# PaddlePaddle/PaddleNLP

Measured on AMD Instinct MI355X. Metric: tokens_per_sec_whole_node_llama3_8b_pretrain, higher is better.
Workload: dtype bf16; 1 GPU; model=llama3-8b, global_batch=8, seq_len=4096, parallelism=single, recompute=False

## Files before the change

### paddlenlp_amd/ops/csrc/flash_attn_bwd_v2.hip

```cpp
#include "launchers.h"
#include "mfma.h"

#define FB2_WAVES 8
#define FB2_BLOCK (FB2_WAVES * 64)

template <int D, bool MASKED = false>
__global__ __launch_bounds__(FB2_BLOCK) void flash_bwd2_dq_kernel(
    const ushort_t* __restrict__ q, const ushort_t* __restrict__ k,
    const ushort_t* __restrict__ v, const ushort_t* __restrict__ dout,
    const float* __restrict__ lse, const float* __restrict__ delta,
    ushort_t* __restrict__ dq, const int* __restrict__ startend,
    FlashStrides rs,
    int B, int Sq, int Skv, int Hq, int Hk, float scale, int causal) {
    constexpr int BLKN = 64;
    constexpr int DSTEPS = D / 16;
    constexpr int NDT = D / 32;
    constexpr int BLKM = FB2_WAVES * 32;

    __shared__ ushort_t k_lds[2][BLKN * D];
    __shared__ ushort_t v_lds[2][BLKN * D];
    __shared__ ushort_t kt_lds[2][D * BLKN];
    __shared__ int se_lds[2][MASKED ? BLKN : 1];

    const int tid = threadIdx.x;
    const int wave = tid >> 6;
    const int lane = tid & 63;
    const int l32 = lane & 31;
    const int hi = lane >> 5;

    int qt, bh;
    xcd_grouped_tile<FA_ORDER_W, false>(qt, bh);
    const int b = bh / Hq, hq = bh % Hq;
    const int hk = hq / (Hq / Hk);
    const int q_base = qt * BLKM;
    const int qw = q_base + wave * 32;
    const int qg = qw + l32;
    const int causal_off = Skv - Sq;

    const long long q_row_stride = rs.q;
    const long long kv_row_stride = rs.kv;
    const long long do_row_stride = (long long)Hq * D;
    const ushort_t* q_ptr = q + (long long)b * Sq * q_row_stride + (long long)hq * D;
    const ushort_t* do_ptr = dout + ((long long)b * Sq * Hq + hq) * D;
    const ushort_t* k_ptr = k + (long long)b * Skv * kv_row_stride + (long long)hk * D;
    const ushort_t* v_ptr = v + (long long)b * Skv * kv_row_stride + (long long)hk * D;

    frag8 aq[DSTEPS], ado[DSTEPS];
    float lse_q = INFINITY, dl_q = 0.f;
    if (qg < Sq) {
#pragma unroll
        for (int kk = 0; kk < DSTEPS; kk++) {
            aq[kk] = *reinterpret_cast<const frag8*>(
                q_ptr + (long long)qg * q_row_stride + kk * 16 + hi * 8);
            ado[kk] = *reinterpret_cast<const frag8*>(
                do_ptr + (long long)qg * do_row_stride + kk * 16 + hi * 8);
        }
        lse_q = lse[((long long)b * Hq + hq) * Sq + qg];
        dl_q = delta[((long long)b * Hq + hq) * Sq + qg];
    } else {
#pragma unroll
        for (int kk = 0; kk < DSTEPS; kk++) { aq[kk] = frag8{0}; ado[kk] = frag8{0}; }
    }

    f32x16 acc_dq[NDT];
#pragma unroll
    for (int n = 0; n < NDT; n++)
#pragma unroll
        for (int r = 0; r < 16; r++) acc_dq[n][r] = 0.f;

    int n_kv_tiles = (Skv + BLKN - 1) / BLKN;
    if (causal) {
        int max_kv = q_base + BLKM - 1 + causal_off;
        int lim = (max_kv + BLKN) / BLKN;
        n_kv_tiles = min(n_kv_tiles, max(lim, 0));
    }

    const int s_rowp = tid >> 4;
    const int s_col = (tid & 15) * 8;
    const int s_row0 = s_rowp * 2;
    short8v sk0, sk1, sv0, sv1;

    auto load_tile = [&](int kv_base) {
        int g0 = kv_base + s_row0;
        sk0 = short8v{0,0,0,0,0,0,0,0}; sk1 = sk0; sv0 = sk0; sv1 = sk0;
        if (g0 < Skv) {
            sk0 = *reinterpret_cast<const short8v*>(k_ptr + (long long)g0 * kv_row_stride + s_col);
            sv0 = *reinterpret_cast<const short8v*>(v_ptr + (long long)g0 * kv_row_stride + s_col);
        }
        if (g0 + 1 < Skv) {
            sk1 = *reinterpret_cast<const short8v*>(k_ptr + (long long)(g0 + 1) * kv_row_stride + s_col);
            sv1 = *reinterpret_cast<const short8v*>(v_ptr + (long long)(g0 + 1) * kv_row_stride + s_col);
        }
    };
    auto write_tile = [&](int buf, int kv_base) {
        if (MASKED && tid < BLKN) {
            int g = kv_base + tid;
            se_lds[buf][tid] =
                (g < Skv) ? startend[(long long)b * Skv + g] : 0;
        }
        *reinterpret_cast<short8v*>(swz<D>(k_lds[buf], s_row0, s_col)) = sk0;
        *reinterpret_cast<short8v*>(swz<D>(k_lds[buf], s_row0 + 1, s_col)) = sk1;
        *reinterpret_cast<short8v*>(swz<D>(v_lds[buf], s_row0, s_col)) = sv0;
        *reinterpret_cast<short8v*>(swz<D>(v_lds[buf], s_row0 + 1, s_col)) = sv1;
#pragma unroll
        for (int j = 0; j < 8; j++) {
            unsigned p32 = ((unsigned)(unsigned short)sk0[j]) |
                           (((unsigned)(unsigned short)sk1[j]) << 16);
            *reinterpret_cast<unsigned*>(swz<BLKN>(kt_lds[buf], s_col + j, s_row0)) = p32;
        }
    };

    auto tile_se_max = [&](int kv_base) -> int {
        int g = kv_base + lane;
        int v = (g < Skv) ? startend[(long long)b * Skv + g] : 0;
#pragma unroll
        for (int off = 32; off; off >>= 1)
            v = max(v, __shfl_xor(v, off, 64));
        return v;
    };

    load_tile(0);
    write_tile(0, 0);
    int se_max_cur = MASKED ? tile_se_max(0) : 0x7fffffff;
    __syncthreads();

    for (int kvt = 0; kvt < n_kv_tiles; kvt++) {
        const int kv_base = kvt * BLKN;
        const int cur = kvt & 1;
        bool wave_skip =
            causal && (kv_base > qw + 31 + causal_off);
        if (MASKED && qw >= se_max_cur) wave_skip = true;

        auto process_sub = [&](int sub) {
            f32x16 st, dp;
#pragma unroll
            for (int r = 0; r < 16; r++) { st[r] = 0.f; dp[r] = 0.f; }
            __builtin_amdgcn_s_setprio(1);
#pragma unroll
            for (int kk = 0; kk < DSTEPS; kk++) {
                frag8 ak = *reinterpret_cast<const frag8*>(
                    swz<D>(k_lds[cur], sub * 32 + l32, kk * 16 + hi * 8));
                frag8 av = *reinterpret_cast<const frag8*>(
                    swz<D>(v_lds[cur], sub * 32 + l32, kk * 16 + hi * 8));
                st = mfma32(ak, aq[kk], st);
                dp = mfma32(av, ado[kk], dp);
            }
            __builtin_amdgcn_s_setprio(0);

#pragma unroll
            for (int r = 0; r < 16; r++) {
                int row = sub * 32 + crow32(r, hi);
                int kvg = kv_base + row;
                bool vis = (kvg < Skv) && (qg < Sq) &&
                           (!causal || kvg <= qg + causal_off);
                if (MASKED) vis = vis && (qg < se_lds[cur][row]);
                float p = vis ? __expf(st[r] * scale - lse_q) : 0.f;
                st[r] = p * (dp[r] - dl_q) * scale;
            }

            __builtin_amdgcn_s_setprio(1);
#pragma unroll
            for (int ksl = 0; ksl < 2; ksl++) {
                const int ks = sub * 2 + ksl;
                frag8 ads = t12_convert(st, ksl * 8);
#pragma unroll
                for (int n = 0; n < NDT; n++) {
                    frag8 bkf = *reinterpret_cast<const frag8*>(
                        swz<BLKN>(kt_lds[cur], n * 32 + l32, ks * 16 + hi * 8));
                    acc_dq[n] = mfma32(ads, bkf, acc_dq[n]);
                }
            }
            __builtin_amdgcn_s_setprio(0);
        };

        if (!wave_skip) process_sub(0);
        int se_max_next = 0x7fffffff;
        bool stage_skip = false;
        if (kvt + 1 < n_kv_tiles) {
            if (MASKED) {
                se_max_next = tile_se_max(kv_base + BLKN);
                stage_skip = (q_base >= se_max_next);
            }
            if (!stage_skip) load_tile(kv_base + BLKN);
        }
        if (!wave_skip) process_sub(1);

        if (kvt + 1 < n_kv_tiles && !stage_skip)
            write_tile(cur ^ 1, kv_base + BLKN);
        if (MASKED) se_max_cur = se_max_next;
        __syncthreads();
    }

#pragma unroll
    for (int r = 0; r < 16; r++) {
        int qrow = qw + crow32(r, hi);
        if (qrow >= Sq) continue;
        ushort_t* dqr = dq + ((long long)b * Sq + qrow) * rs.dq + (long long)hq * D;
#pragma unroll
        for (int n = 0; n < NDT; n++)
            dqr[n * 32 + l32] = f32_to_bf16(acc_dq[n][r]);
    }
}

template <int D, bool MASKED = false>
__global__ __launch_bounds__(FB2_BLOCK, 1) void flash_bwd2_dkv_kernel(
    const ushort_t* __restrict__ q, const ushort_t* __restrict__ k,
    const ushort_t* __restrict__ v, const ushort_t* __restrict__ dout,
    const float* __restrict__ lse, const float* __restrict__ delta,
    ushort_t* __restrict__ dk, ushort_t* __restrict__ dv,
    const int* __restrict__ startend,
    FlashStrides rs,
    int B, int Sq, int Skv, int Hq, int Hk, float scale, int causal) {
    static_assert(D == 128, "the dual-use image is laid out for 128-column tiles");
    constexpr int BLKQ = 64;
    constexpr int DSTEPS = D / 16;
    constexpr int NDT = D / 32;
    constexpr int BLKKV = FB2_WAVES * 32;

    __shared__ __attribute__((aligned(16))) ushort_t qd_lds[2][2][BLKQ * D];
    __shared__ float ld_lds[2][2][BLKQ];

    const int tid = threadIdx.x;
    const int wave = __builtin_amdgcn_readfirstlane(tid >> 6);
    const int lane = tid & 63;
    const int l32 = lane & 31;
    const int hi = lane >> 5;

    int kvt, bh;
    xcd_grouped_tile<FA_ORDER_W, true>(kvt, bh);
    const int b = bh / Hk, hk = bh % Hk;
    const int G = Hq / Hk;
    const int kv_base = kvt * BLKKV;
    const int kvw = kv_base + wave * 32;
    const int kvg_lane = kvw + l32;
    const int causal_off = Skv - Sq;
    __shared__ int blk_max_lds[MASKED ? FB2_WAVES : 1];
    int kv_end_lane = 0x7fffffff;
    int wave_max_end = 0x7fffffff;
    if (MASKED) {
        kv_end_lane = (kvg_lane < Skv)
            ? startend[(long long)b * Skv + kvg_lane] : 0;
        wave_max_end = kv_end_lane;
#pragma unroll
        for (int off = 32; off; off >>= 1)
            wave_max_end = max(wave_max_end,
                               __shfl_xor(wave_max_end, off, 64));
        wave_max_end = __builtin_amdgcn_readfirstlane(wave_max_end);
        if (lane == 0) blk_max_lds[wave] = wave_max_end;
    }

    const long long do_row_stride = (long long)Hq * D;
    const ushort_t* k_ptr = k + (long long)b * Skv * rs.kv + (long long)hk * D;
    const ushort_t* v_ptr = v + (long long)b * Skv * rs.kv + (long long)hk * D;

    frag8 bk[DSTEPS], bv[DSTEPS];
    if (kvg_lane < Skv) {
#pragma unroll
        for (int kk = 0; kk < DSTEPS; kk++) {
            bk[kk] = *reinterpret_cast<const frag8*>(
                k_ptr + (long long)kvg_lane * rs.kv + kk * 16 + hi * 8);
            bv[kk] = *reinterpret_cast<const frag8*>(
                v_ptr + (long long)kvg_lane * rs.kv + kk * 16 + hi * 8);
        }
    } else {
#pragma unroll
        for (int kk = 0; kk < DSTEPS; kk++) { bk[kk] = frag8{0}; bv[kk] = frag8{0}; }
    }

    f32x16 acc_dk[NDT], acc_dv[NDT];
#pragma unroll
    for (int n = 0; n < NDT; n++)
#pragma unroll
        for (int r = 0; r < 16; r++) { acc_dk[n][r] = 0.f; acc_dv[n][r] = 0.f; }

    int qt0 = 0;
    if (causal) qt0 = max(0, (kv_base - causal_off) / BLKQ);
    int qt_end = (Sq + BLKQ - 1) / BLKQ;
    if (MASKED) {
        __syncthreads();
        int block_max_end = blk_max_lds[0];
#pragma unroll
        for (int w = 1; w < FB2_WAVES; w++)
            block_max_end = max(block_max_end, blk_max_lds[w]);
        block_max_end = __builtin_amdgcn_readfirstlane(block_max_end);
        if (block_max_end < Sq)
            qt_end = (max(block_max_end, 0) + BLKQ - 1) / BLKQ;
    }
    const int n_tiles = G * max(qt_end - qt0, 0);

    auto issue_tile = [&](int g, int qt, int buf) {
        const int hq = hk * G + g;
        const long long do_off = ((long long)b * Sq * Hq + hq) * D;
        const long long q_off = (long long)b * Sq * rs.q + (long long)hq * D;
        const int q_tb = qt * BLKQ;
        const int ln = fresh_lane_id();
#pragma unroll
        for (int i = 0; i < 2; i++) {
            const int piece = wave * 2 + i;
            const int src_row = min(q_tb + img_fill_row(piece, ln), Sq - 1);
            const int chunk = img_fill_chunk(piece, ln) * 8;
            lds_dma16(q + (q_off + (long long)src_row * rs.q + chunk),
                      &qd_lds[buf][0][piece * 512]);
            lds_dma16(dout + (do_off + (long long)src_row * do_row_stride + chunk),
                      &qd_lds[buf][1][piece * 512]);
        }
        if (wave < 2) {
            const float* row = (wave == 0 ? lse : delta) +
                               ((long long)b * Hq + hq) * Sq;
            lds_dma4(row + min(q_tb + ln, Sq - 1), &ld_lds[buf][wave][0]);
        }
    };

    int g_next = 0, qt_next = qt0;
    auto advance_next = [&]() {
        if (++qt_next == qt_end) { qt_next = qt0; g_next++; }
    };
#pragma unroll
    for (int kk = 0; kk < DSTEPS; kk++)
        asm volatile("" :: "v"(bk[kk]), "v"(bv[kk]));
    if (n_tiles > 0) { issue_tile(g_next, qt_next, 0); advance_next(); }

    int qt = qt0;
    for (int t = 0; t < n_tiles; t++) {
        const int cur = t & 1;
        lds_dma_wait_all();
        __syncthreads();
        if (t + 1 < n_tiles) { issue_tile(g_next, qt_next, cur ^ 1); advance_next(); }

        const int q_tb = qt * BLKQ;
        const ushort_t* q_img = qd_lds[cur][0];
        const ushort_t* do_img = qd_lds[cur][1];
        const int lane_t = fresh_lane_id();
        bool wave_skip =
            causal && (q_tb + BLKQ - 1 + causal_off < kvw);
        if (MASKED && q_tb >= wave_max_end) wave_skip = true;

        if (!wave_skip) {
#pragma unroll 1
            for (int sub = 0; sub < 2; sub++) {
                f32x16 st, dp;
#pragma unroll
                for (int r = 0; r < 16; r++) { st[r] = 0.f; dp[r] = 0.f; }
                __builtin_amdgcn_s_setprio(1);
#pragma unroll
                for (int kk = 0; kk < DSTEPS; kk++) {
                    frag8 aqf = img_row_frag(q_img, sub * 32 + l32, kk, hi);
                    frag8 adf = img_row_frag(do_img, sub * 32 + l32, kk, hi);
                    st = mfma32(aqf, bk[kk], st);
                    dp = mfma32(adf, bv[kk], dp);
                }
                __builtin_amdgcn_s_setprio(0);

#pragma unroll
                for (int r = 0; r < 16; r++) {
                    int qrow = sub * 32 + crow32(r, hi);
                    int qgl = q_tb + qrow;
                    float ls = ld_lds[cur][0][qrow];
                    float dl = ld_lds[cur][1][qrow];
                    bool vis = (qgl < Sq) && (kvg_lane < Skv) &&
                               (!causal || kvg_lane <= qgl + causal_off);
                    if (MASKED) vis = vis && (qgl < kv_end_lane);
                    float p = (vis && ls != INFINITY)
                                  ? __expf(st[r] * scale - ls) : 0.f;
                    st[r] = p;
                    dp[r] = p * (dp[r] - dl) * scale;
                }

                __builtin_amdgcn_s_setprio(1);
#pragma unroll
                for (int ksl = 0; ksl < 2; ksl++) {
                    const int ks = sub * 2 + ksl;
                    frag8 apt = t12_convert(st, ksl * 8);
                    frag8 ads = t12_convert(dp, ksl * 8);
#pragma unroll
                    for (int n = 0; n < NDT; n++) {
                        frag8 bdo = img_tr_frag(do_img, ks, n, lane_t);
                        frag8 bq = img_tr_frag(q_img, ks, n, lane_t);
                        acc_dv[n] = mfma32(apt, bdo, acc_dv[n]);
                        acc_dk[n] = mfma32(ads, bq, acc_dk[n]);
                    }
                }
                __builtin_amdgcn_s_setprio(0);
            }
        }
        if (++qt == qt_end) qt = qt0;
    }

#pragma unroll
    for (int r = 0; r < 16; r++) {
        int kvr = kvw + crow32(r, hi);
        if (kvr >= Skv) continue;
        long long base = ((long long)b * Skv + kvr) * rs.dkv + (long long)hk * D;
#pragma unroll
        for (int n = 0; n < NDT; n++) {
            dk[base + n * 32 + l32] = f32_to_bf16(acc_dk[n][r]);
            dv[base + n * 32 + l32] = f32_to_bf16(acc_dv[n][r]);
        }
    }
}

__global__ __launch_bounds__(64) void lds_image_probe(
    const ushort_t* __restrict__ X, ushort_t* __restrict__ out_row,
    ushort_t* __restrict__ out_tr) {
    __shared__ __attribute__((aligned(16))) ushort_t img[64 * 128];
    const int lane = threadIdx.x;
    const int l32 = lane & 31, hi = lane >> 5;
#pragma unroll 1
    for (int piece = 0; piece < 16; piece++)
        lds_dma16(X + img_fill_row(piece, lane) * 128 + img_fill_chunk(piece, lane) * 8,
                  &img[piece * 512]);
    lds_dma_wait_all();
    __syncthreads();
    for (int sub = 0; sub < 2; sub++)
        for (int kk = 0; kk < 8; kk++) {
            frag8 f = img_row_frag(img, sub * 32 + l32, kk, hi);
            *reinterpret_cast<frag8*>(
                out_row + (sub * 32 + l32) * 128 + kk * 16 + hi * 8) = f;
        }
    for (int ks = 0; ks < 4; ks++)
        for (int n = 0; n < 4; n++) {
            frag8 f = img_tr_frag(img, ks, n, lane);
#pragma unroll
            for (int j = 0; j < 8; j++)
                out_tr[(ks * 16 + hi * 8 + j) * 128 + n * 32 + l32] = (ushort_t)f[j];
        }
}

void launch_lds_image_probe(const void* X, void* out_row, void* out_tr,
                            hipStream_t stream) {
    hipLaunchKernelGGL(lds_image_probe, dim3(1), dim3(64), 0, stream,
                       (const ushort_t*)X, (ushort_t*)out_row, (ushort_t*)out_tr);
}

bool launch_flash_bwd2(const void* dout, const void* q, const void* k, const void* v,
                       const void* o, const float* lse, float* delta,
                       void* dq, void* dk, void* dv,
                       int B, int Sq, int Skv, int Hq, int Hk, int D,
                       float scale, bool causal, hipStream_t stream, int parts,
                       const FlashStrides* strides) {
    if (D != 128 || (Hq % Hk) != 0) return false;
    const FlashStrides rs = strides ? *strides : flash_contiguous_strides(Hq, Hk, D);
    if (parts & FLASH_BWD_DELTA)
        launch_flash_bwd_delta(dout, o, delta, B, Sq, Hq, D, stream);
    if (parts & FLASH_BWD_DQ) {
        dim3 gq((Sq + 255) / 256, B * Hq);
        hipLaunchKernelGGL((flash_bwd2_dq_kernel<128, false>), gq, dim3(FB2_BLOCK), 0, stream,
                           (const ushort_t*)q, (const ushort_t*)k, (const ushort_t*)v,
                           (const ushort_t*)dout, lse, delta, (ushort_t*)dq,
                           (const int*)nullptr, rs,
                           B, Sq, Skv, Hq, Hk, scale, causal ? 1 : 0);
    }
    if (parts & FLASH_BWD_DKV) {
        dim3 gkv((Skv + 255) / 256, B * Hk);
        hipLaunchKernelGGL((flash_bwd2_dkv_kernel<128, false>), gkv, dim3(FB2_BLOCK), 0, stream,
                           (const ushort_t*)q, (const ushort_t*)k, (const ushort_t*)v,
                           (const ushort_t*)dout, lse, delta, (ushort_t*)dk, (ushort_t*)dv,
                           (const int*)nullptr, rs,
                           B, Sq, Skv, Hq, Hk, scale, causal ? 1 : 0);
    }
    return true;
}

bool launch_flash_bwd2_mask(const void* dout, const void* q, const void* k,
                            const void* v, const void* o, const float* lse,
                            float* delta, void* dq, void* dk, void* dv,
                            const int* startend,
                            int B, int Sq, int Skv, int Hq, int Hk, int D,
                            float scale, hipStream_t stream,
                            const FlashStrides* strides) {
    if (D != 128 || (Hq % Hk) != 0) return false;
    const FlashStrides rs = strides ? *strides : flash_contiguous_strides(Hq, Hk, D);
    launch_flash_bwd_delta(dout, o, delta, B, Sq, Hq, D, stream);
    dim3 gq((Sq + 255) / 256, B * Hq);
    hipLaunchKernelGGL((flash_bwd2_dq_kernel<128, true>), gq, dim3(FB2_BLOCK), 0, stream,
                       (const ushort_t*)q, (const ushort_t*)k, (const ushort_t*)v,
                       (const ushort_t*)dout, lse, delta, (ushort_t*)dq, startend, rs,
                       B, Sq, Skv, Hq, Hk, scale, 1);
    dim3 gkv((Skv + 255) / 256, B * Hk);
    hipLaunchKernelGGL((flash_bwd2_dkv_kernel<128, true>), gkv, dim3(FB2_BLOCK), 0, stream,
                       (const ushort_t*)q, (const ushort_t*)k, (const ushort_t*)v,
                       (const ushort_t*)dout, lse, delta, (ushort_t*)dk, (ushort_t*)dv,
                       startend, rs, B, Sq, Skv, Hq, Hk, scale, 1);
    return true;
}
```

### paddlenlp_amd/ops/csrc/flash_attn_v2.hip

```cpp
#include "launchers.h"
#include "mfma.h"

#define FA2_WAVES 8
#define FA2_BLOCK (FA2_WAVES * 64)
#define FA2_BLKN 64
#define FA2_QW 32
#define FA2_BLKM (FA2_WAVES * FA2_QW)
#define DEFER_THR 8.0f

__global__ void mfma32_layout_probe(const ushort_t* A, const ushort_t* B, float* C) {
    int l = threadIdx.x;
    int l32 = l & 31, hi = l >> 5;
    frag8 a, b;
#pragma unroll
    for (int j = 0; j < 8; j++) {
        a[j] = (short)A[l32 * 16 + hi * 8 + j];
        b[j] = (short)B[(hi * 8 + j) * 32 + l32];
    }
    f32x16 c;
#pragma unroll
    for (int r = 0; r < 16; r++) c[r] = 0.f;
    c = mfma32(a, b, c);
#pragma unroll
    for (int r = 0; r < 16; r++) C[crow32(r, hi) * 32 + l32] = c[r];
}

__global__ void permlane_probe(int* out0, int* out1) {
    int l = threadIdx.x;
    auto r = __builtin_amdgcn_permlane32_swap((unsigned)l, (unsigned)(1000 + l),
                                              false, false);
    out0[l] = (int)r[0];
    out1[l] = (int)r[1];
}

template <int D, bool MASKED = false>
__global__ __launch_bounds__(FA2_BLOCK) void flash_fwd2_kernel(
    const ushort_t* __restrict__ q,
    const ushort_t* __restrict__ k,
    const ushort_t* __restrict__ v,
    ushort_t* __restrict__ o,
    float* __restrict__ lse,
    const int* __restrict__ startend,
    FlashStrides rs,
    int B, int Sq, int Skv, int Hq, int Hk, float scale, int causal) {
    constexpr int DSTEPS = D / 16;
    constexpr int NDT = D / 32;
    constexpr int KVT = FA2_BLKN / 32;

    __shared__ ushort_t k_lds[2][FA2_BLKN * D];
    __shared__ ushort_t vt_lds[2][D * FA2_BLKN];
    __shared__ int se_lds[2][MASKED ? FA2_BLKN : 1];

    const int tid = threadIdx.x;
    const int wave = tid >> 6;
    const int lane = tid & 63;
    const int l32 = lane & 31;
    const int hi = lane >> 5;

    int qt, bh;
    xcd_grouped_tile<FA_ORDER_W, false>(qt, bh);
    const int b = bh / Hq, hq = bh % Hq;
    const int hk = hq / (Hq / Hk);
    const int q_base = qt * FA2_BLKM;
    const int qw = q_base + wave * FA2_QW;
    const int qg = qw + l32;
    const int causal_off = Skv - Sq;

    const long long q_row_stride = rs.q;
    const long long kv_row_stride = rs.kv;
    const long long o_row_stride = (long long)Hq * D;
    const ushort_t* q_ptr = q + (long long)b * Sq * q_row_stride + (long long)hq * D;
    const ushort_t* k_ptr = k + (long long)b * Skv * kv_row_stride + (long long)hk * D;
    const ushort_t* v_ptr = v + (long long)b * Skv * kv_row_stride + (long long)hk * D;

    frag8 aq[DSTEPS];
    if (qg < Sq) {
#pragma unroll
        for (int kk = 0; kk < DSTEPS; kk++)
            aq[kk] = *reinterpret_cast<const frag8*>(
                q_ptr + (long long)qg * q_row_stride + kk * 16 + hi * 8);
    } else {
#pragma unroll
        for (int kk = 0; kk < DSTEPS; kk++) aq[kk] = frag8{0};
    }

    float m_run = -INFINITY, l_run = 0.f;
    f32x16 acc_o[NDT];
#pragma unroll
    for (int n = 0; n < NDT; n++)
#pragma unroll
        for (int r = 0; r < 16; r++) acc_o[n][r] = 0.f;

    int n_kv_tiles = (Skv + FA2_BLKN - 1) / FA2_BLKN;
    if (causal) {
        int max_kv = q_base + FA2_BLKM - 1 + causal_off;
        int lim = (max_kv + FA2_BLKN) / FA2_BLKN;
        n_kv_tiles = min(n_kv_tiles, max(lim, 0));
    }

    const int s_rowp = tid >> 4;
    const int s_col = (tid & 15) * 8;
    const int s_row0 = s_rowp * 2;
    short8v sk0, sk1, sv0, sv1;

    auto load_tile = [&](int kv_base) {
        int g0 = kv_base + s_row0;
        sk0 = short8v{0,0,0,0,0,0,0,0}; sk1 = sk0; sv0 = sk0; sv1 = sk0;
        if (g0 < Skv) {
            sk0 = *reinterpret_cast<const short8v*>(k_ptr + (long long)g0 * kv_row_stride + s_col);
            sv0 = *reinterpret_cast<const short8v*>(v_ptr + (long long)g0 * kv_row_stride + s_col);
        }
        if (g0 + 1 < Skv) {
            sk1 = *reinterpret_cast<const short8v*>(k_ptr + (long long)(g0 + 1) * kv_row_stride + s_col);
            sv1 = *reinterpret_cast<const short8v*>(v_ptr + (long long)(g0 + 1) * kv_row_stride + s_col);
        }
    };
    auto write_tile = [&](int buf, int kv_base) {
        if (MASKED && tid < FA2_BLKN) {
            int g = kv_base + tid;
            se_lds[buf][tid] =
                (g < Skv) ? startend[(long long)b * Skv + g] : 0;
        }
        *reinterpret_cast<short8v*>(swz<D>(k_lds[buf], s_row0, s_col)) = sk0;
        *reinterpret_cast<short8v*>(swz<D>(k_lds[buf], s_row0 + 1, s_col)) = sk1;
#pragma unroll
        for (int j = 0; j < 8; j++) {
            unsigned p32 = ((unsigned)(unsigned short)sv0[j]) |
                           (((unsigned)(unsigned short)sv1[j]) << 16);
            *reinterpret_cast<unsigned*>(swz<FA2_BLKN>(vt_lds[buf], s_col + j, s_row0)) = p32;
        }
    };

    auto tile_bounds = [&](int kv_base, int& mn_out) -> int {
        int g = kv_base + lane;
        int v = (g < Skv) ? startend[(long long)b * Skv + g] : 0;
        int mx = v, mn = (g < Skv) ? v : 0x7fffffff;
#pragma unroll
        for (int off = 32; off; off >>= 1) {
            mx = max(mx, __shfl_xor(mx, off, 64));
            mn = min(mn, __shfl_xor(mn, off, 64));
        }
        mn_out = mn;
        return mx;
    };

    load_tile(0);
    write_tile(0, 0);
    int se_min_cur = 0, se_max_cur = 0x7fffffff;
    if (MASKED) se_max_cur = tile_bounds(0, se_min_cur);
    __syncthreads();

    for (int kvt = 0; kvt < n_kv_tiles; kvt++) {
        const int kv_base = kvt * FA2_BLKN;
        const int cur = kvt & 1;
        bool wave_skip =
            causal && (kv_base > qw + FA2_QW - 1 + causal_off);
        if (MASKED && qw >= se_max_cur) wave_skip = true;

        f32x16 st[KVT];
        if (!wave_skip) {
#pragma unroll
            for (int nt = 0; nt < KVT; nt++)
#pragma unroll
                for (int r = 0; r < 16; r++) st[nt][r] = 0.f;
            __builtin_amdgcn_s_setprio(1);
#pragma unroll
            for (int kk = 0; kk < DSTEPS; kk++) {
#pragma unroll
                for (int nt = 0; nt < KVT; nt++) {
                    frag8 ak = *reinterpret_cast<const frag8*>(
                        swz<D>(k_lds[cur], nt * 32 + l32, kk * 16 + hi * 8));
                    st[nt] = mfma32(ak, aq[kk], st[nt]);
                }
            }
            __builtin_amdgcn_s_setprio(0);
        }

        int se_min_next = 0, se_max_next = 0x7fffffff;
        bool stage_skip = false;
        if (kvt + 1 < n_kv_tiles) {
            if (MASKED) {
                se_max_next = tile_bounds(kv_base + FA2_BLKN, se_min_next);
                stage_skip = (q_base >= se_max_next);
            }
            if (!stage_skip) load_tile(kv_base + FA2_BLKN);
        }

        if (!wave_skip) {
            const bool full_tile =
                (kv_base + FA2_BLKN <= Skv) &&
                (!causal || (kv_base + FA2_BLKN - 1 <= qw + causal_off)) &&
                (!MASKED || (qw + FA2_QW - 1 < se_min_cur));
            if (full_tile) {
#pragma unroll
                for (int nt = 0; nt < KVT; nt++)
#pragma unroll
                    for (int r = 0; r < 16; r++) st[nt][r] *= scale;
            } else {
#pragma unroll
                for (int nt = 0; nt < KVT; nt++)
#pragma unroll
                    for (int r = 0; r < 16; r++) {
                        int row = nt * 32 + crow32(r, hi);
                        int kvg = kv_base + row;
                        bool vis = (kvg < Skv) &&
                                   (!causal || kvg <= qg + causal_off);
                        if (MASKED) vis = vis && (qg < se_lds[cur][row]);
                        st[nt][r] = vis ? st[nt][r] * scale : -INFINITY;
                    }
            }

            float pm = -INFINITY;
#pragma unroll
            for (int nt = 0; nt < KVT; nt++)
#pragma unroll
                for (int r = 0; r < 16; r++) pm = fmaxf(pm, st[nt][r]);
            {
                union { float f; unsigned u; } x{pm};
                auto rr = __builtin_amdgcn_permlane32_swap(x.u, x.u, false, false);
                union { unsigned u; float f; } a{rr[0]}, c{rr[1]};
                pm = fmaxf(a.f, c.f);
            }

            bool grew = pm > m_run + DEFER_THR ||
                        (m_run == -INFINITY && pm > -INFINITY);
            if (__any(grew)) {
                float m_new = fmaxf(m_run, pm);
                float alpha = (m_run == -INFINITY)
                                  ? 0.f
                                  : __expf(m_run - m_new);
                if (m_new == -INFINITY) alpha = 1.f;
                l_run *= alpha;
                m_run = m_new;
#pragma unroll
                for (int r = 0; r < 16; r++) {
                    float ar = __shfl(alpha, crow32(r, hi), 64);
#pragma unroll
                    for (int n = 0; n < NDT; n++) acc_o[n][r] *= ar;
                }
            }

            float ps = 0.f;
#pragma unroll
            for (int nt = 0; nt < KVT; nt++)
#pragma unroll
                for (int r = 0; r < 16; r++) {
                    float s = st[nt][r];
                    float p = (s == -INFINITY) ? 0.f : __expf(s - m_run);
                    st[nt][r] = p;
                    ps += p;
                }
            {
                union { float f; unsigned u; } x{ps};
                auto rr = __builtin_amdgcn_permlane32_swap(x.u, x.u, false, false);
                union { unsigned u; float f; } a{rr[0]}, c{rr[1]};
                ps = a.f + c.f;
            }
            l_run += ps;

            __builtin_amdgcn_s_setprio(1);
#pragma unroll
            for (int ks = 0; ks < FA2_BLKN / 16; ks++) {
                frag8 pa = t12_convert(st[ks >> 1], (ks & 1) * 8);
#pragma unroll
                for (int n = 0; n < NDT; n++) {
                    frag8 bv = *reinterpret_cast<const frag8*>(
                        swz<FA2_BLKN>(vt_lds[cur], n * 32 + l32, ks * 16 + hi * 8));
                    acc_o[n] = mfma32(pa, bv, acc_o[n]);
                }
            }
            __builtin_amdgcn_s_setprio(0);
        }

        if (kvt + 1 < n_kv_tiles && !stage_skip)
            write_tile(cur ^ 1, kv_base + FA2_BLKN);
        if (MASKED) { se_max_cur = se_max_next; se_min_cur = se_min_next; }
        __syncthreads();
    }

    float inv_l = (l_run > 0.f) ? 1.0f / l_run : 0.f;
#pragma unroll
    for (int r = 0; r < 16; r++) {
        int qrow = qw + crow32(r, hi);
        if (qrow >= Sq) continue;
        float il = __shfl(inv_l, crow32(r, hi), 64);
        ushort_t* orow = o + ((long long)b * Sq + qrow) * o_row_stride + (long long)hq * D;
#pragma unroll
        for (int n = 0; n < NDT; n++)
            orow[n * 32 + l32] = f32_to_bf16(acc_o[n][r] * il);
    }
    if (hi == 0 && qg < Sq) {
        float lv = (l_run > 0.f) ? (m_run + __logf(l_run)) : -INFINITY;
        lse[((long long)b * Hq + hq) * Sq + qg] = lv;
    }
}

void launch_mfma32_probe(const void* A, const void* B, float* C, hipStream_t stream) {
    hipLaunchKernelGGL(mfma32_layout_probe, dim3(1), dim3(64), 0, stream,
                       (const ushort_t*)A, (const ushort_t*)B, C);
}

void launch_permlane_probe(int* out0, int* out1, hipStream_t stream) {
    hipLaunchKernelGGL(permlane_probe, dim3(1), dim3(64), 0, stream, out0, out1);
}

bool launch_flash_fwd2(const void* q, const void* k, const void* v, void* o,
                       float* lse, int B, int Sq, int Skv, int Hq, int Hk,
                       int D, float scale, bool causal, hipStream_t stream,
                       const FlashStrides* strides) {
    if (D != 128 || (Hq % Hk) != 0) return false;
    const FlashStrides rs = strides ? *strides : flash_contiguous_strides(Hq, Hk, D);
    dim3 grid((Sq + FA2_BLKM - 1) / FA2_BLKM, B * Hq);
    hipLaunchKernelGGL((flash_fwd2_kernel<128, false>), grid, dim3(FA2_BLOCK), 0, stream,
                       (const ushort_t*)q, (const ushort_t*)k, (const ushort_t*)v,
                       (ushort_t*)o, lse, (const int*)nullptr, rs,
                       B, Sq, Skv, Hq, Hk, scale, causal ? 1 : 0);
    return true;
}

bool launch_flash_fwd2_mask(const void* q, const void* k, const void* v,
                            void* o, float* lse, const int* startend,
                            int B, int Sq, int Skv, int Hq, int Hk,
                            int D, float scale, hipStream_t stream,
                            const FlashStrides* strides) {
    if (D != 128 || (Hq % Hk) != 0) return false;
    const FlashStrides rs = strides ? *strides : flash_contiguous_strides(Hq, Hk, D);
    dim3 grid((Sq + FA2_BLKM - 1) / FA2_BLKM, B * Hq);
    hipLaunchKernelGGL((flash_fwd2_kernel<128, true>), grid, dim3(FA2_BLOCK), 0,
                       stream, (const ushort_t*)q, (const ushort_t*)k,
                       (const ushort_t*)v, (ushort_t*)o, lse, startend, rs,
                       B, Sq, Skv, Hq, Hk, scale, 1);
    return true;
}
```

### paddlenlp_amd/ops/csrc/launchers.h

```cpp
#pragma once

#include <hip/hip_runtime_api.h>

#include <stdexcept>
#include <string>

[[noreturn]] inline void unsupported_head_dim(const char* op, int D) {
    throw std::runtime_error(std::string(op) + ": no kernel for head dim " +
                             std::to_string(D));
}

void launch_rms_norm_fwd(const void* x, const void* delta, const void* w, void* h,
                         void* y, float* invrms,
                         long long rows, int H, float eps, hipStream_t stream);
int rms_norm_bwd_partials(long long rows, int H, bool* needs_zero);
void launch_rms_norm_bwd(const void* dy, const void* x, const void* dh, const void* w,
                         const float* invrms, void* dx, float* dw_partial,
                         float* dw32, void* dw, bool dw_is_bf16,
                         long long rows, int H, int P, hipStream_t stream);
void launch_rope(const void* x, void* out, const float* cos_t, const float* sin_t,
                 long long n_rows, int H, int D, int S, bool backward,
                 hipStream_t stream);
void launch_rope_packed(void* qkv, const float* cos_t, const float* sin_t,
                        long long n_tokens, int Hq, int Hk, int D, int S,
                        bool backward, hipStream_t stream);
void launch_swiglu_fwd(const void* x, void* y, long long N, int I, hipStream_t stream);
void launch_swiglu_bwd(const void* dy, const void* x, void* dx, long long N, int I,
                       hipStream_t stream);
void launch_ce_fwd(const void* logits, const long long* labels, float* loss,
                   float* maxlse, long long N, int V, long long ignore_index,
                   hipStream_t stream);
void launch_ce_bwd(const float* dloss, const void* logits, const long long* labels,
                   const float* maxlse, void* dlogits, long long N, int V,
                   long long ignore_index, hipStream_t stream);

struct AdamWChunk {
    void* param;
    const void* grad;
    float* m;
    float* v;
    float* master;
    long long offset;
    long long n;
    int is_bf16;
};
void launch_adamw(const AdamWChunk* dev_chunks, int n_chunks,
                  float lr, float beta1, float beta2, float eps, float wd,
                  float bias1, float bias2, hipStream_t stream);

void launch_mfma_probe(const void* A, const void* B, float* C, hipStream_t stream);
void launch_flash_fwd(const void* q, const void* k, const void* v, void* o,
                      float* lse, int B, int Sq, int Skv, int Hq, int Hk, int D,
                      float scale, bool causal, bool force_v1, hipStream_t stream);
void launch_flash_bwd(const void* dout, const void* q, const void* k, const void* v,
                      const void* o, const float* lse, float* delta,
                      void* dq, void* dk, void* dv,
                      int B, int Sq, int Skv, int Hq, int Hk, int D,
                      float scale, bool causal, bool force_v1, hipStream_t stream);
void launch_flash_fwd_mask(const void* q, const void* k, const void* v, void* o,
                           float* lse, const int* startend,
                           int B, int Sq, int Skv, int Hq, int Hk, int D,
                           float scale, hipStream_t stream);
void launch_flash_bwd_mask(const void* dout, const void* q, const void* k, const void* v,
                           const void* o, const float* lse, float* delta,
                           void* dq, void* dk, void* dv, const int* startend,
                           int B, int Sq, int Skv, int Hq, int Hk, int D,
                           float scale, hipStream_t stream);
void launch_flash_bwd_delta(const void* dout, const void* o, float* delta,
                            int B, int Sq, int Hq, int D, hipStream_t stream);

struct FlashStrides { int q, kv, dq, dkv; };
inline FlashStrides flash_contiguous_strides(int Hq, int Hk, int D) {
    return {Hq * D, Hk * D, Hq * D, Hk * D};
}
inline FlashStrides flash_packed_strides(int Hq, int Hk, int D) {
    int w = (Hq + 2 * Hk) * D;
    return {w, w, w, w};
}
void launch_mfma32_probe(const void* A, const void* B, float* C, hipStream_t stream);
void launch_permlane_probe(int* out0, int* out1, hipStream_t stream);
void launch_lds_image_probe(const void* X, void* out_row, void* out_tr,
                            hipStream_t stream);
bool launch_flash_fwd2(const void* q, const void* k, const void* v, void* o,
                       float* lse, int B, int Sq, int Skv, int Hq, int Hk,
                       int D, float scale, bool causal, hipStream_t stream,
                       const FlashStrides* strides = nullptr);
bool launch_flash_fwd2_mask(const void* q, const void* k, const void* v,
                            void* o, float* lse, const int* startend,
                            int B, int Sq, int Skv, int Hq, int Hk,
                            int D, float scale, hipStream_t stream,
                            const FlashStrides* strides = nullptr);
enum { FLASH_BWD_DELTA = 1, FLASH_BWD_DQ = 2, FLASH_BWD_DKV = 4, FLASH_BWD_ALL = 7 };
bool launch_flash_bwd2(const void* dout, const void* q, const void* k, const void* v,
                       const void* o, const float* lse, float* delta,
                       void* dq, void* dk, void* dv,
                       int B, int Sq, int Skv, int Hq, int Hk, int D,
                       float scale, bool causal, hipStream_t stream,
                       int parts = FLASH_BWD_ALL,
                       const FlashStrides* strides = nullptr);
bool launch_flash_bwd2_mask(const void* dout, const void* q, const void* k,
                            const void* v, const void* o, const float* lse,
                            float* delta, void* dq, void* dk, void* dv,
                            const int* startend,
                            int B, int Sq, int Skv, int Hq, int Hk, int D,
                            float scale, hipStream_t stream,
                            const FlashStrides* strides = nullptr);

int paged_decode_nsplit(int B, int Hk);
void launch_paged_decode_attn(const void* q, const void* k_cache, const void* v_cache,
                              const float* k_scale, const float* v_scale,
                              const int* block_table, const int* seq_lens, void* out,
                              float* partials, int nsplit,
                              int B, int Hq, int Hk, int D, int block_size,
                              int max_blocks, float scale, int cache_mode,
                              hipStream_t stream);
bool launch_paged_decode_attn3(const void* q, const void* k_cache, const void* v_cache,
                               const float* k_scale, const float* v_scale,
                               const int* block_table, const int* seq_lens, void* out,
                               float* partials, int nsplit,
                               int B, int Hq, int Hk, int D, int block_size,
                               int max_blocks, float scale, int cache_mode,
                               hipStream_t stream);
void launch_rope_cache_append(const void* qkv, void* q_out, void* k_cache, void* v_cache,
                              float* k_scale, float* v_scale,
                              const int* block_table, const int* seq_lens_before,
                              const float* cos_t, const float* sin_t,
                              int B, int T, int Hq, int Hk, int D, int block_size,
                              int max_blocks, const int* token_counts,
                              int cache_mode, hipStream_t stream);

bool paged_append_plan(int B, int T, int Hq, int Hk, int D, int r_tiles,
                       int* R, int* nrg, int* nsplit);
bool launch_paged_append_attn(const void* q, const void* k_cache, const void* v_cache,
                              const float* k_scale, const float* v_scale,
                              const int* block_table, const int* seq_lens_before,
                              const int* token_counts, void* out, float* partials,
                              int r_tiles, int B, int T, int Hq, int Hk, int D,
                              int block_size, int max_blocks, float scale,
                              int cache_mode, hipStream_t stream);

void launch_wint8_gemv(const void* x, const void* wq, const float* scale, void* y,
                       int M, int N, int K, hipStream_t stream);
void launch_fp8_rowwise_quant(const void* x, void* y, float* scales,
                              long long R, int K, hipStream_t stream);
int skinny_gemm_ksplit(int N, int K, int ksplit_req);
void launch_skinny_gemm(const void* x, const void* w, float* partial, void* y,
                        int M, int N, int K, int ksplit, hipStream_t stream);

void launch_repetition_penalty(void* logits, const long long* pre_ids,
                               const int* pre_lens, const float* rep_pen,
                               int B, long long V, int max_len, hipStream_t s);
void launch_topp_sample(const void* logits, const float* temperature,
                        const float* top_p, const float* uniform,
                        const long long* ban_eos, int n_ban,
                        const int* cur_lens, const int* min_lens,
                        long long* out, int B, long long V, hipStream_t s);
void launch_decode_update(long long* tokens, signed char* stop_flags,
                          const signed char* active, long long* pre_ids,
                          int* pre_lens, int* seq_lens,
                          const long long* eos_ids, int n_eos,
                          int* not_need_stop, const int* max_new,
                          long long pad_id, int B, int max_len, hipStream_t s);
void launch_block_step(int* block_table, int* seq_lens, signed char* stop_flags,
                       signed char* active, int* free_list, int* free_count,
                       signed char* is_block_step, int B, int block_size,
                       int max_blocks, hipStream_t s);
```

Baseline: 21610 tokens/s.

## Stage flash-attention K/V tiles via direct global-to-LDS DMA into a shared dual-use image

Replaces the register-staged K/V tile loads (global load, then swizzled LDS store plus a separately written transposed copy) in the forward and dQ backward flash kernels with direct global-to-LDS DMA into a single image. That image serves both row-major and transposed fragment reads, which drops the extra transposed buffer and the VGPR round-trip. The mask bounds are also DMA'd into a three-slot ring so tile min/max come from LDS. The intent is to cut LDS footprint, register pressure and load-path instructions and to overlap the next tile's fetch with compute. The cost is a wait-all plus barrier at the top of every iteration, an alignment guard that returns false for misaligned inputs, and a hard restriction to D=128.

New measurement: 21920 tokens/s, median of 6. +1.4%, better.

```diff
diff --git a/paddlenlp_amd/ops/csrc/flash_attn_bwd_v2.hip b/paddlenlp_amd/ops/csrc/flash_attn_bwd_v2.hip
--- a/paddlenlp_amd/ops/csrc/flash_attn_bwd_v2.hip
+++ b/paddlenlp_amd/ops/csrc/flash_attn_bwd_v2.hip
@@ -12,18 +12,17 @@
     ushort_t* __restrict__ dq, const int* __restrict__ startend,
     FlashStrides rs,
     int B, int Sq, int Skv, int Hq, int Hk, float scale, int causal) {
+    static_assert(D == 128, "the dual-use image is laid out for 128-column tiles");
     constexpr int BLKN = 64;
     constexpr int DSTEPS = D / 16;
     constexpr int NDT = D / 32;
     constexpr int BLKM = FB2_WAVES * 32;
 
-    __shared__ ushort_t k_lds[2][BLKN * D];
-    __shared__ ushort_t v_lds[2][BLKN * D];
-    __shared__ ushort_t kt_lds[2][D * BLKN];
-    __shared__ int se_lds[2][MASKED ? BLKN : 1];
+    __shared__ __attribute__((aligned(16))) ushort_t kv_lds[2][2][BLKN * D];
+    __shared__ int se_lds[3][MASKED ? BLKN : 1];
 
     const int tid = threadIdx.x;
-    const int wave = tid >> 6;
+    const int wave = __builtin_amdgcn_readfirstlane(tid >> 6);
     const int lane = tid & 63;
     const int l32 = lane & 31;
     const int hi = lane >> 5;
@@ -75,58 +74,67 @@
         n_kv_tiles = min(n_kv_tiles, max(lim, 0));
     }
 
-    const int s_rowp = tid >> 4;
-    const int s_col = (tid & 15) * 8;
-    const int s_row0 = s_rowp * 2;
-    short8v sk0, sk1, sv0, sv1;
-
-    auto load_tile = [&](int kv_base) {
-        int g0 = kv_base + s_row0;
-        sk0 = short8v{0,0,0,0,0,0,0,0}; sk1 = sk0; sv0 = sk0; sv1 = sk0;
-        if (g0 < Skv) {
-            sk0 = *reinterpret_cast<const short8v*>(k_ptr + (long long)g0 * kv_row_stride + s_col);
-            sv0 = *reinterpret_cast<const short8v*>(v_ptr + (long long)g0 * kv_row_stride + s_col);
-        }
-        if (g0 + 1 < Skv) {
-            sk1 = *reinterpret_cast<const short8v*>(k_ptr + (long long)(g0 + 1) * kv_row_stride + s_col);
-            sv1 = *reinterpret_cast<const short8v*>(v_ptr + (long long)(g0 + 1) * kv_row_stride + s_col);
+    auto issue_tile = [&](int kv_base, int buf) {
+        const int ln = fresh_lane_id();
+#pragma unroll
+        for (int i = 0; i < 2; i++) {
+            const int piece = wave * 2 + i;
+            const int src_row = min(kv_base + img_fill_row(piece, ln), Skv - 1);
+            const long long off = (long long)src_row * kv_row_stride +
+                                  img_fill_chunk(piece, ln) * 8;
+            lds_dma16(k_ptr + off, &kv_lds[buf][0][piece * 512]);
+            lds_dma16(v_ptr + off, &kv_lds[buf][1][piece * 512]);
         }
     };
-    auto write_tile = [&](int buf, int kv_base) {
-        if (MASKED && tid < BLKN) {
-            int g = kv_base + tid;
-            se_lds[buf][tid] =
-                (g < Skv) ? startend[(long long)b * Skv + g] : 0;
-        }
-        *reinterpret_cast<short8v*>(swz<D>(k_lds[buf], s_row0, s_col)) = sk0;
-        *reinterpret_cast<short8v*>(swz<D>(k_lds[buf], s_row0 + 1, s_col)) = sk1;
-        *reinterpret_cast<short8v*>(swz<D>(v_lds[buf], s_row0, s_col)) = sv0;
-        *reinterpret_cast<short8v*>(swz<D>(v_lds[buf], s_row0 + 1, s_col)) = sv1;
-#pragma unroll
-        for (int j = 0; j < 8; j++) {
-            unsigned p32 = ((unsigned)(unsigned short)sk0[j]) |
-                           (((unsigned)(unsigned short)sk1[j]) << 16);
-            *reinterpret_cast<unsigned*>(swz<BLKN>(kt_lds[buf], s_col + j, s_row0)) = p32;
+    auto issue_bounds = [&](int tile, int slot) {
+        if (MASKED && wave == 0) {
+            const int ln = fresh_lane_id();
+            lds_dma4(startend + (long long)b * Skv + min(tile * BLKN + ln, Skv - 1),
+                     &se_lds[slot][0]);
         }
     };
-
-    auto tile_se_max = [&](int kv_base) -> int {
-        int g = kv_base + lane;
-        int v = (g < Skv) ? startend[(long long)b * Skv + g] : 0;
+    auto tile_se_max = [&](int slot) -> int {
+        int v = se_lds[slot][lane];
 #pragma unroll
         for (int off = 32; off; off >>= 1)
             v = max(v, __shfl_xor(v, off, 64));
-        return v;
+        return __builtin_amdgcn_readfirstlane(v);
     };
 
-    load_tile(0);
-    write_tile(0, 0);
-    int se_max_cur = MASKED ? tile_se_max(0) : 0x7fffffff;
-    __syncthreads();
+#pragma unroll
+    for (int kk = 0; kk < DSTEPS; kk++)
+        asm volatile("" :: "v"(aq[kk]), "v"(ado[kk]));
+    asm volatile("" :: "v"(lse_q), "v"(dl_q));
+    if (n_kv_tiles > 0) {
+        issue_tile(0, 0);
+        issue_bounds(0, 0);
+        if (n_kv_tiles > 1) issue_bounds(1, 1);
+    }
+    int se_max_cur = 0x7fffffff;
+    int se_slot = 0;
 
     for (int kvt = 0; kvt < n_kv_tiles; kvt++) {
         const int kv_base = kvt * BLKN;
         const int cur = kvt & 1;
+        lds_dma_wait_all();
+        __syncthreads();
+        const int se_slot_next = (se_slot == 2) ? 0 : se_slot + 1;
+        if (MASKED && kvt == 0) se_max_cur = tile_se_max(0);
+        int se_max_next = 0x7fffffff;
+        if (kvt + 1 < n_kv_tiles) {
+            bool stage_skip = false;
+            if (MASKED) {
+                se_max_next = tile_se_max(se_slot_next);
+                stage_skip = (q_base >= se_max_next);
+            }
+            if (!stage_skip) issue_tile(kv_base + BLKN, cur ^ 1);
+            if (kvt + 2 < n_kv_tiles)
+                issue_bounds(kvt + 2, (se_slot_next == 2) ? 0 : se_slot_next + 1);
+        }
+        const ushort_t* k_img = kv_lds[cur][0];
+        const ushort_t* v_img = kv_lds[cur][1];
+        const int lane_t = fresh_lane_id();
+
         bool wave_skip =
             causal && (kv_base > qw + 31 + causal_off);
         if (MASKED && qw >= se_max_cur) wave_skip = true;
@@ -138,10 +146,8 @@
             __builtin_amdgcn_s_setprio(1);
 #pragma unroll
             for (int kk = 0; kk < DSTEPS; kk++) {
-                frag8 ak = *reinterpret_cast<const frag8*>(
-                    swz<D>(k_lds[cur], sub * 32 + l32, kk * 16 + hi * 8));
-                frag8 av = *reinterpret_cast<const frag8*>(
-                    swz<D>(v_lds[cur], sub * 32 + l32, kk * 16 + hi * 8));
+                frag8 ak = img_row_frag(k_img, sub * 32 + l32, kk, hi);
+                frag8 av = img_row_frag(v_img, sub * 32 + l32, kk, hi);
                 st = mfma32(ak, aq[kk], st);
                 dp = mfma32(av, ado[kk], dp);
             }
@@ -153,7 +159,7 @@
                 int kvg = kv_base + row;
                 bool vis = (kvg < Skv) && (qg < Sq) &&
                            (!causal || kvg <= qg + causal_off);
-                if (MASKED) vis = vis && (qg < se_lds[cur][row]);
+                if (MASKED) vis = vis && (qg < se_lds[se_slot][row]);
                 float p = vis ? __expf(st[r] * scale - lse_q) : 0.f;
                 st[r] = p * (dp[r] - dl_q) * scale;
             }
@@ -165,30 +171,19 @@
                 frag8 ads = t12_convert(st, ksl * 8);
 #pragma unroll
                 for (int n = 0; n < NDT; n++) {
-                    frag8 bkf = *reinterpret_cast<const frag8*>(
-                        swz<BLKN>(kt_lds[cur], n * 32 + l32, ks * 16 + hi * 8));
+                    frag8 bkf = img_tr_frag(k_img, ks, n, lane_t);
                     acc_dq[n] = mfma32(ads, bkf, acc_dq[n]);
                 }
             }
             __builtin_amdgcn_s_setprio(0);
         };
 
-        if (!wave_skip) process_sub(0);
-        int se_max_next = 0x7fffffff;
-        bool stage_skip = false;
-        if (kvt + 1 < n_kv_tiles) {
-            if (MASKED) {
-                se_max_next = tile_se_max(kv_base + BLKN);
-                stage_skip = (q_base >= se_max_next);
-            }
-            if (!stage_skip) load_tile(kv_base + BLKN);
-        }
-        if (!wave_skip) process_sub(1);
-
-        if (kvt + 1 < n_kv_tiles && !stage_skip)
-            write_tile(cur ^ 1, kv_base + BLKN);
+        if (!wave_skip) {
+            process_sub(0);
+            process_sub(1);
+        }
         if (MASKED) se_max_cur = se_max_next;
-        __syncthreads();
+        se_slot = se_slot_next;
     }
 
 #pragma unroll
@@ -440,6 +435,9 @@
                        const FlashStrides* strides) {
     if (D != 128 || (Hq % Hk) != 0) return false;
     const FlashStrides rs = strides ? *strides : flash_contiguous_strides(Hq, Hk, D);
+    if (!flash_dma_aligned(q, rs.q) || !flash_dma_aligned(k, rs.kv) ||
+        !flash_dma_aligned(v, rs.kv) || !flash_dma_aligned(dout, Hq * D))
+        return false;
     if (parts & FLASH_BWD_DELTA)
         launch_flash_bwd_delta(dout, o, delta, B, Sq, Hq, D, stream);
     if (parts & FLASH_BWD_DQ) {
@@ -470,6 +468,9 @@
                             const FlashStrides* strides) {
     if (D != 128 || (Hq % Hk) != 0) return false;
     const FlashStrides rs = strides ? *strides : flash_contiguous_strides(Hq, Hk, D);
+    if (!flash_dma_aligned(q, rs.q) || !flash_dma_aligned(k, rs.kv) ||
+        !flash_dma_aligned(v, rs.kv) || !flash_dma_aligned(dout, Hq * D))
+        return false;
     launch_flash_bwd_delta(dout, o, delta, B, Sq, Hq, D, stream);
     dim3 gq((Sq + 255) / 256, B * Hq);
     hipLaunchKernelGGL((flash_bwd2_dq_kernel<128, true>), gq, dim3(FB2_BLOCK), 0, stream,
diff --git a/paddlenlp_amd/ops/csrc/flash_attn_v2.hip b/paddlenlp_amd/ops/csrc/flash_attn_v2.hip
--- a/paddlenlp_amd/ops/csrc/flash_attn_v2.hip
+++ b/paddlenlp_amd/ops/csrc/flash_attn_v2.hip
@@ -43,16 +43,16 @@
     const int* __restrict__ startend,
     FlashStrides rs,
     int B, int Sq, int Skv, int Hq, int Hk, float scale, int causal) {
+    static_assert(D == 128, "the dual-use image is laid out for 128-column tiles");
     constexpr int DSTEPS = D / 16;
     constexpr int NDT = D / 32;
     constexpr int KVT = FA2_BLKN / 32;
 
-    __shared__ ushort_t k_lds[2][FA2_BLKN * D];
-    __shared__ ushort_t vt_lds[2][D * FA2_BLKN];
-    __shared__ int se_lds[2][MASKED ? FA2_BLKN : 1];
+    __shared__ __attribute__((aligned(16))) ushort_t kv_lds[2][2][FA2_BLKN * D];
+    __shared__ int se_lds[3][MASKED ? FA2_BLKN : 1];
 
     const int tid = threadIdx.x;
-    const int wave = tid >> 6;
+    const int wave = __builtin_amdgcn_readfirstlane(tid >> 6);
     const int lane = tid & 63;
     const int l32 = lane & 31;
     const int hi = lane >> 5;
@@ -98,61 +98,68 @@
         n_kv_tiles = min(n_kv_tiles, max(lim, 0));
     }
 
-    const int s_rowp = tid >> 4;
-    const int s_col = (tid & 15) * 8;
-    const int s_row0 = s_rowp * 2;
-    short8v sk0, sk1, sv0, sv1;
-
-    auto load_tile = [&](int kv_base) {
-        int g0 = kv_base + s_row0;
-        sk0 = short8v{0,0,0,0,0,0,0,0}; sk1 = sk0; sv0 = sk0; sv1 = sk0;
-        if (g0 < Skv) {
-            sk0 = *reinterpret_cast<const short8v*>(k_ptr + (long long)g0 * kv_row_stride + s_col);
-            sv0 = *reinterpret_cast<const short8v*>(v_ptr + (long long)g0 * kv_row_stride + s_col);
-        }
-        if (g0 + 1 < Skv) {
-            sk1 = *reinterpret_cast<const short8v*>(k_ptr + (long long)(g0 + 1) * kv_row_stride + s_col);
-            sv1 = *reinterpret_cast<const short8v*>(v_ptr + (long long)(g0 + 1) * kv_row_stride + s_col);
+    auto issue_tile = [&](int kv_base, int buf) {
+        const int ln = fresh_lane_id();
+#pragma unroll
+        for (int i = 0; i < 2; i++) {
+            const int piece = wave * 2 + i;
+            const int src_row = min(kv_base + img_fill_row(piece, ln), Skv - 1);
+            const long long off = (long long)src_row * kv_row_stride +
+                                  img_fill_chunk(piece, ln) * 8;
+            lds_dma16(k_ptr + off, &kv_lds[buf][0][piece * 512]);
+            lds_dma16(v_ptr + off, &kv_lds[buf][1][piece * 512]);
         }
     };
-    auto write_tile = [&](int buf, int kv_base) {
-        if (MASKED && tid < FA2_BLKN) {
-            int g = kv_base + tid;
-            se_lds[buf][tid] =
-                (g < Skv) ? startend[(long long)b * Skv + g] : 0;
-        }
-        *reinterpret_cast<short8v*>(swz<D>(k_lds[buf], s_row0, s_col)) = sk0;
-        *reinterpret_cast<short8v*>(swz<D>(k_lds[buf], s_row0 + 1, s_col)) = sk1;
-#pragma unroll
-        for (int j = 0; j < 8; j++) {
-            unsigned p32 = ((unsigned)(unsigned short)sv0[j]) |
-                           (((unsigned)(unsigned short)sv1[j]) << 16);
-            *reinterpret_cast<unsigned*>(swz<FA2_BLKN>(vt_lds[buf], s_col + j, s_row0)) = p32;
+    auto issue_bounds = [&](int tile, int slot) {
+        if (MASKED && wave == 0) {
+            const int ln = fresh_lane_id();
+            lds_dma4(startend + (long long)b * Skv + min(tile * FA2_BLKN + ln, Skv - 1),
+                     &se_lds[slot][0]);
         }
     };
-
-    auto tile_bounds = [&](int kv_base, int& mn_out) -> int {
-        int g = kv_base + lane;
-        int v = (g < Skv) ? startend[(long long)b * Skv + g] : 0;
-        int mx = v, mn = (g < Skv) ? v : 0x7fffffff;
+    auto tile_bounds = [&](int slot, int& mn_out) -> int {
+        int mx = se_lds[slot][lane], mn = mx;
 #pragma unroll
         for (int off = 32; off; off >>= 1) {
             mx = max(mx, __shfl_xor(mx, off, 64));
             mn = min(mn, __shfl_xor(mn, off, 64));
         }
-        mn_out = mn;
-        return mx;
+        mn_out = __builtin_amdgcn_readfirstlane(mn);
+        return __builtin_amdgcn_readfirstlane(mx);
     };
 
-    load_tile(0);
-    write_tile(0, 0);
+#pragma unroll
+    for (int kk = 0; kk < DSTEPS; kk++) asm volatile("" :: "v"(aq[kk]));
+    if (n_kv_tiles > 0) {
+        issue_tile(0, 0);
+        issue_bounds(0, 0);
+        if (n_kv_tiles > 1) issue_bounds(1, 1);
+    }
     int se_min_cur = 0, se_max_cur = 0x7fffffff;
-    if (MASKED) se_max_cur = tile_bounds(0, se_min_cur);
-    __syncthreads();
+    int se_slot = 0;
 
     for (int kvt = 0; kvt < n_kv_tiles; kvt++) {
         const int kv_base = kvt * FA2_BLKN;
         const int cur = kvt & 1;
+        lds_dma_wait_all();
+        __syncthreads();
+        const int se_slot_next = (se_slot == 2) ? 0 : se_slot + 1;
+        if (MASKED && kvt == 0) se_max_cur = tile_bounds(0, se_min_cur);
+        int se_min_next = 0, se_max_next = 0x7fffffff;
+        if (kvt + 1 < n_kv_tiles) {
+            bool stage_skip = false;
+            if (MASKED) {
+                se_max_next = tile_bounds(se_slot_next, se_min_next);
+                stage_skip = (q_base >= se_max_next);
+            }
+            if (!stage_skip) issue_tile(kv_base + FA2_BLKN, cur ^ 1);
+            if (kvt + 2 < n_kv_tiles)
+                issue_bounds(kvt + 2, (se_slot_next == 2) ? 0 : se_slot_next + 1);
+        }
+        const ushort_t* k_img = kv_lds[cur][0];
+        const ushort_t* v_img = kv_lds[cur][1];
+        const int lane_t = fresh_lane_id();
+
         bool wave_skip =
             causal && (kv_base > qw + FA2_QW - 1 + causal_off);
         if (MASKED && qw >= se_max_cur) wave_skip = true;
@@ -168,25 +175,12 @@
             for (int kk = 0; kk < DSTEPS; kk++) {
 #pragma unroll
                 for (int nt = 0; nt < KVT; nt++) {
-                    frag8 ak = *reinterpret_cast<const frag8*>(
-                        swz<D>(k_lds[cur], nt * 32 + l32, kk * 16 + hi * 8));
+                    frag8 ak = img_row_frag(k_img, nt * 32 + l32, kk, hi);
                     st[nt] = mfma32(ak, aq[kk], st[nt]);
                 }
             }
             __builtin_amdgcn_s_setprio(0);
-        }
-
-        int se_min_next = 0, se_max_next = 0x7fffffff;
-        bool stage_skip = false;
-        if (kvt + 1 < n_kv_tiles) {
-            if (MASKED) {
-                se_max_next = tile_bounds(kv_base + FA2_BLKN, se_min_next);
-                stage_skip = (q_base >= se_max_next);
-            }
-            if (!stage_skip) load_tile(kv_base + FA2_BLKN);
-        }
-
-        if (!wave_skip) {
+
             const bool full_tile =
                 (kv_base + FA2_BLKN <= Skv) &&
                 (!causal || (kv_base + FA2_BLKN - 1 <= qw + causal_off)) &&
@@ -205,7 +199,7 @@
                         int kvg = kv_base + row;
                         bool vis = (kvg < Skv) &&
                                    (!causal || kvg <= qg + causal_off);
-                        if (MASKED) vis = vis && (qg < se_lds[cur][row]);
+                        if (MASKED) vis = vis && (qg < se_lds[se_slot][row]);
                         st[nt][r] = vis ? st[nt][r] * scale : -INFINITY;
                     }
             }
@@ -264,18 +258,15 @@
                 frag8 pa = t12_convert(st[ks >> 1], (ks & 1) * 8);
 #pragma unroll
                 for (int n = 0; n < NDT; n++) {
-                    frag8 bv = *reinterpret_cast<const frag8*>(
-                        swz<FA2_BLKN>(vt_lds[cur], n * 32 + l32, ks * 16 + hi * 8));
+                    frag8 bv = img_tr_frag(v_img, ks, n, lane_t);
                     acc_o[n] = mfma32(pa, bv, acc_o[n]);
                 }
             }
             __builtin_amdgcn_s_setprio(0);
         }
 
-        if (kvt + 1 < n_kv_tiles && !stage_skip)
-            write_tile(cur ^ 1, kv_base + FA2_BLKN);
         if (MASKED) { se_max_cur = se_max_next; se_min_cur = se_min_next; }
-        __syncthreads();
+        se_slot = se_slot_next;
     }
 
     float inv_l = (l_run > 0.f) ? 1.0f / l_run : 0.f;
@@ -310,6 +301,7 @@
                        const FlashStrides* strides) {
     if (D != 128 || (Hq % Hk) != 0) return false;
     const FlashStrides rs = strides ? *strides : flash_contiguous_strides(Hq, Hk, D);
+    if (!flash_dma_aligned(k, rs.kv) || !flash_dma_aligned(v, rs.kv)) return false;
     dim3 grid((Sq + FA2_BLKM - 1) / FA2_BLKM, B * Hq);
     hipLaunchKernelGGL((flash_fwd2_kernel<128, false>), grid, dim3(FA2_BLOCK), 0, stream,
                        (const ushort_t*)q, (const ushort_t*)k, (const ushort_t*)v,
@@ -325,6 +317,7 @@
                             const FlashStrides* strides) {
     if (D != 128 || (Hq % Hk) != 0) return false;
     const FlashStrides rs = strides ? *strides : flash_contiguous_strides(Hq, Hk, D);
+    if (!flash_dma_aligned(k, rs.kv) || !flash_dma_aligned(v, rs.kv)) return false;
     dim3 grid((Sq + FA2_BLKM - 1) / FA2_BLKM, B * Hq);
     hipLaunchKernelGGL((flash_fwd2_kernel<128, true>), grid, dim3(FA2_BLOCK), 0,
                        stream, (const ushort_t*)q, (const ushort_t*)k,
diff --git a/paddlenlp_amd/ops/csrc/launchers.h b/paddlenlp_amd/ops/csrc/launchers.h
--- a/paddlenlp_amd/ops/csrc/launchers.h
+++ b/paddlenlp_amd/ops/csrc/launchers.h
@@ -2,6 +2,7 @@
 
 #include <hip/hip_runtime_api.h>
 
+#include <cstdint>
 #include <stdexcept>
 #include <string>
 
@@ -76,6 +77,9 @@
 inline FlashStrides flash_packed_strides(int Hq, int Hk, int D) {
     int w = (Hq + 2 * Hk) * D;
     return {w, w, w, w};
+}
+inline bool flash_dma_aligned(const void* p, int row_stride) {
+    return reinterpret_cast<uintptr_t>(p) % 16 == 0 && row_stride % 8 == 0;
 }
 void launch_mfma32_probe(const void* A, const void* B, float* C, hipStream_t stream);
 void launch_permlane_probe(int* out0, int* out1, hipStream_t stream);
```
